# marcomistretta/incremental_multimodal_medical_learning_II

Hardware: AMD Instinct MI355X
Metric: contrastive train-step images/sec at global batch 1024; 1/2/4/8-GPU scaling (higher is better)
Workload: dtype bf16x3

## Files before the change

### incremental_multimodal_medical_learning_ii_amd/csrc/bert.hip

```cpp
#include "cxrk.h"
#include "cxrk_common.h"
#include "dropout.h"

using namespace cxrk;

namespace {

constexpr int LN_MAXV = 16;

template <bool EMBED>
__global__ __launch_bounds__(256) void ln_fwd_kernel(const float* __restrict__ x, const float* __restrict__ res,
                                                     const long* __restrict__ ids, const float* __restrict__ word,
                                                     const float* __restrict__ pos, const float* __restrict__ type,
                                                     const float* __restrict__ gamma, const float* __restrict__ beta,
                                                     float eps, long rows, int H, int L, float* __restrict__ y,
                                                     float* __restrict__ xhat, float* __restrict__ rstd_out) {
  const long row = (long)blockIdx.x * 4 + (threadIdx.x >> 6);
  if (row >= rows) return;
  const int lane = threadIdx.x & 63;
  float v[LN_MAXV];
  float s = 0.f;
  const float* xr = EMBED ? word + ids[row] * H : x + row * H;
  const float* rr = EMBED ? pos + (row % L) * H : (res ? res + row * H : nullptr);
#pragma unroll
// ... 317 lines not shown
    const int row = i / d4, c4 = i % d4;
    *reinterpret_cast<float4*>(Qs + row * ALD + c4 * 4) = *reinterpret_cast<const float4*>(base + (long)row * ld + c4 * 4);
    *reinterpret_cast<float4*>(Ks + row * ALD + c4 * 4) = *reinterpret_cast<const float4*>(base + (long)row * ld + nH * dH + c4 * 4);
    *reinterpret_cast<float4*>(Vs + row * ALD + c4 * 4) = *reinterpret_cast<const float4*>(base + (long)row * ld + 2 * nH * dH + c4 * 4);
  }
  __syncthreads();
  const int LP = L + 1;
  const int nb = (L + 1) / 2;
  for (int blk = threadIdx.x; blk < nb * nb; blk += 256) {
    const int i0 = 2 * (blk / nb), j0 = 2 * (blk % nb);
    const int i1 = min(i0 + 1, L - 1), j1 = min(j0 + 1, L - 1);
    float o[2][2];
    dot2x2(Qs, Ks, ALD, d4, i0, i1, j0, j1, o);
    const bool m0 = mask && mask[(long)b * L + j0] == 0, m1 = mask && mask[(long)b * L + j1] == 0;
    constexpr float MASKED = -3.4028234663852886e38f;
    Ps[i0 * LP + j0] = m0 ? MASKED : o[0][0] * scale;
    Ps[i0 * LP + j1] = m1 ? MASKED : o[0][1] * scale;
    Ps[i1 * LP + j0] = m0 ? MASKED : o[1][0] * scale;
    Ps[i1 * LP + j1] = m1 ? MASKED : o[1][1] * scale;
  }
  __syncthreads();
  {
    const int row = threadIdx.x >> 2, sub = threadIdx.x & 3;
    if (row < L) {
      float m = -INFINITY;
      for (int j = sub; j < L; j += 4) m = fmaxf(m, Ps[row * LP + j]);
      m = fmaxf(m, __shfl_xor(m, 1, 64)); m = fmaxf(m, __shfl_xor(m, 2, 64));
      float sum = 0.f;
      for (int j = sub; j < L; j += 4) { const float p = expf(Ps[row * LP + j] - m); Ps[row * LP + j] = p; sum += p; }
      sum += __shfl_xor(sum, 1, 64); sum += __shfl_xor(sum, 2, 64);
      const float inv = 1.0f / sum;
      for (int j = sub; j < L; j += 4) {
        const float p = Ps[row * LP + j] * inv;
        Ps[row * LP + j] = p;
        if (probs) probs[(((long)b * nH + hd) * L + row) * L + j] = p;
      }
    }
  }
  __syncthreads();
  if constexpr (DROP) {
    const int nj4 = (L + 3) / 4;
    for (int e = threadIdx.x; e < L * nj4; e += 256)
      drop_prob_row4(dk, Ps + (e / nj4) * LP, 0, e % nj4, L, (unsigned)(dk.row_offset + b), e / nj4, hd);
    __syncthreads();
  }
  const long obase = (long)b * L * (nH * dH) + hd * dH;
  float* out = ctx + obase;
  for (int blk = threadIdx.x; blk < nb * d4; blk += 256) {
    const int i0 = 2 * (blk / d4), dq = blk % d4;
    const int i1 = min(i0 + 1, L - 1);
    float4 a0 = make_float4(0.f, 0.f, 0.f, 0.f), a1 = a0;
    for (int j = 0; j < L; ++j) {
      const float4 v = *reinterpret_cast<const float4*>(Vs + j * ALD + dq * 4);
      fma4(a0, Ps[i0 * LP + j], v); fma4(a1, Ps[i1 * LP + j], v);
    }
    if (ctxp) {
      const float v0[4] = {a0.x, a0.y, a0.z, a0.w}, v1[4] = {a1.x, a1.y, a1.z, a1.w};
      planes_store4(ctxp, ctxplane, obase + (long)i0 * (nH * dH) + dq * 4, v0);
      if (i0 + 1 < L) planes_store4(ctxp, ctxplane, obase + (long)i1 * (nH * dH) + dq * 4, v1);
    } else {
      *reinterpret_cast<float4*>(out + (long)i0 * (nH * dH) + dq * 4) = a0;
      if (i0 + 1 < L) *reinterpret_cast<float4*>(out + (long)i1 * (nH * dH) + dq * 4) = a1;
    }
  }
}

template <bool DROP = false>
__global__ __launch_bounds__(256) void attn_bwd_kernel(const float* __restrict__ qkv, const float* __restrict__ probs,
                                                       const float* __restrict__ dctx, int L, int nH, int dH, float scale,
                                                       float* __restrict__ dqkv, unsigned short* __restrict__ dqkvp, long dqkvplane,
                                                       DropKey dk) {
  extern __shared__ __attribute__((aligned(16))) float smem[];
  const int ALD = dH + 4;
  float* Qs = smem; float* Ks = Qs + L * ALD; float* Vs = Ks + L * ALD; float* Os = Vs + L * ALD;
  float* Ps = Os + L * ALD; float* Ds = Ps + L * (L + 1);
  float* Pv = DROP ? Ds + L * (L + 1) : Ps;
  const int b = blockIdx.x / nH, hd = blockIdx.x % nH;
  const int ld = 3 * nH * dH;
  const int d4 = dH / 4;
  const float* base = qkv + (long)b * L * ld + hd * dH;
  const float* dob = dctx + (long)b * L * (nH * dH) + hd * dH;
  for (int i = threadIdx.x; i < L * d4; i += 256) {
    const int row = i / d4, c4 = i % d4;
    *reinterpret_cast<float4*>(Qs + row * ALD + c4 * 4) = *reinterpret_cast<const float4*>(base + (long)row * ld + c4 * 4);
    *reinterpret_cast<float4*>(Ks + row * ALD + c4 * 4) = *reinterpret_cast<const float4*>(base + (long)row * ld + nH * dH + c4 * 4);
    *reinterpret_cast<float4*>(Vs + row * ALD + c4 * 4) = *reinterpret_cast<const float4*>(base + (long)row * ld + 2 * nH * dH + c4 * 4);
    *reinterpret_cast<float4*>(Os + row * ALD + c4 * 4) = *reinterpret_cast<const float4*>(dob + (long)row * (nH * dH) + c4 * 4);
  }
  const int LP = L + 1;
  const float* pb = probs + ((long)b * nH + hd) * L * L;
  for (int e = threadIdx.x; e < L * L; e += 256) Ps[(e / L) * LP + (e % L)] = pb[e];
  __syncthreads();
  const int nb = (L + 1) / 2;
  for (int blk = threadIdx.x; blk < nb * nb; blk += 256) {
    const int i0 = 2 * (blk / nb), j0 = 2 * (blk % nb);
    const int i1 = min(i0 + 1, L - 1), j1 = min(j0 + 1, L - 1);
    float o[2][2];
    dot2x2(Os, Vs, ALD, d4, i0, i1, j0, j1, o);
    Ds[i0 * LP + j0] = o[0][0]; Ds[i0 * LP + j1] = o[0][1]; Ds[i1 * LP + j0] = o[1][0]; Ds[i1 * LP + j1] = o[1][1];
  }
  __syncthreads();
  if constexpr (DROP) {
    const int nj4 = (L + 3) / 4;
    for (int e = threadIdx.x; e < L * nj4; e += 256) {
      const int row = e / nj4, g = e % nj4;
      float f[4];
      drop_factors4(dk, (unsigned)g, (unsigned)(dk.row_offset + b), (unsigned)row | ((unsigned)hd << 16), f);
#pragma unroll
      for (int q = 0; q < 4; ++q) {
        const int j = 4 * g + q;
        if (j < L) { Ds[row * LP + j] *= f[q]; Pv[row * LP + j] = Ps[row * LP + j] * f[q]; }
      }
    }
    __syncthreads();
  }
  {
    const int row = threadIdx.x >> 2, sub = threadIdx.x & 3;
    if (row < L) {
      float t = 0.f;
      for (int j = sub; j < L; j += 4) t += Ds[row * LP + j] * Ps[row * LP + j];
      t += __shfl_xor(t, 1, 64); t += __shfl_xor(t, 2, 64);
      for (int j = sub; j < L; j += 4) Ds[row * LP + j] = Ps[row * LP + j] * (Ds[row * LP + j] - t) * scale;
    }
  }
  __syncthreads();
  const long qbase = (long)b * L * ld + hd * dH;
  float* dq = dqkv + qbase;
  auto put = [&](long off, const float4& v) {
    if (dqkvp) { const float t[4] = {v.x, v.y, v.z, v.w}; planes_store4(dqkvp, dqkvplane, qbase + off, t); }
    else *reinterpret_cast<float4*>(dq + off) = v;
  };
  for (int blk = threadIdx.x; blk < nb * d4; blk += 256) {
    const int i0 = 2 * (blk / d4), c = blk % d4;
    const int i1 = min(i0 + 1, L - 1);
    const float4 z = make_float4(0.f, 0.f, 0.f, 0.f);
    float4 q0 = z, q1 = z, k0 = z, k1 = z, v0 = z, v1 = z;
    for (int j = 0; j < L; ++j) {
      const float4 kj = *reinterpret_cast<const float4*>(Ks + j * ALD + c * 4);
      const float4 qj = *reinterpret_cast<const float4*>(Qs + j * ALD + c * 4);
      const float4 oj = *reinterpret_cast<const float4*>(Os + j * ALD + c * 4);
      fma4(q0, Ds[i0 * LP + j], kj); fma4(q1, Ds[i1 * LP + j], kj);
      fma4(k0, Ds[j * LP + i0], qj); fma4(k1, Ds[j * LP + i1], qj);
      fma4(v0, Pv[j * LP + i0], oj); fma4(v1, Pv[j * LP + i1], oj);
    }
    const long o0 = (long)i0 * ld + c * 4;
    put(o0, q0); put(o0 + nH * dH, k0); put(o0 + 2 * nH * dH, v0);
    if (i0 + 1 < L) {
      const long o1 = (long)i1 * ld + c * 4;
      put(o1, q1); put(o1 + nH * dH, k1); put(o1 + 2 * nH * dH, v1);
    }
  }
}

constexpr int ALONG = 512;
constexpr int TQ = 32, TK = 64;

__device__ __forceinline__ void load_rows(float* dst, const float* src, long ld, int r0, int nrows, int L, int d4, int ALD) {
  for (int i = threadIdx.x; i < nrows * d4; i += 256) {
    const int row = i / d4, c4 = i % d4;
    float4 v = make_float4(0.f, 0.f, 0.f, 0.f);
    if (r0 + row < L) v = *reinterpret_cast<const float4*>(src + (long)(r0 + row) * ld + c4 * 4);
    *reinterpret_cast<float4*>(dst + row * ALD + c4 * 4) = v;
  }
}
__device__ __forceinline__ void dot1x8(const float* X, const float* Y, int ALD, int d4n, int i, int jg, float (&o)[8]) {
#pragma unroll
  for (int c = 0; c < 8; ++c) o[c] = 0.f;
  const float4* x = reinterpret_cast<const float4*>(X + i * ALD);
  for (int d = 0; d < d4n; ++d) {
    const float4 a = x[d];
#pragma unroll
    for (int c = 0; c < 8; ++c) o[c] = dot4(a, reinterpret_cast<const float4*>(Y + (jg + 8 * c) * ALD)[d], o[c]);
  }
}

template <bool DROP = false>
__global__ __launch_bounds__(256) void attn_fwd_long_kernel(const float* __restrict__ qkv, const long* __restrict__ mask, int L, int nH,
                                                            int dH, float scale, float* __restrict__ ctx,
                                                            unsigned short* __restrict__ ctxp, long ctxplane, float* __restrict__ probs,
                                                            DropKey dk) {
  extern __shared__ __attribute__((aligned(16))) float smem[];
  const int ALD = dH + 4, d4 = dH / 4, LP = L + 1;
  float* Qs = smem; float* Ts = Qs + TQ * ALD; float* Ps = Ts + TK * ALD;
  const int nqt = (L + TQ - 1) / TQ;
  const int qt = blockIdx.x % nqt, bh = blockIdx.x / nqt;
  const int b = bh / nH, hd = bh % nH;
  const int ld = 3 * nH * dH;
  const float* base = qkv + (long)b * L * ld + hd * dH;
  const int q0 = qt * TQ;
  const int i = threadIdx.x >> 3, sub = threadIdx.x & 7;
  constexpr float MASKED = -3.4028234663852886e38f;
  load_rows(Qs, base, ld, q0, TQ, L, d4, ALD);
  for (int k0 = 0; k0 < L; k0 += TK) {
    __syncthreads();
    load_rows(Ts, base + nH * dH, ld, k0, TK, L, d4, ALD);
    __syncthreads();
    float o[8];
    dot1x8(Qs, Ts, ALD, d4, i, sub, o);
#pragma unroll
    for (int c = 0; c < 8; ++c) {
      const int j = k0 + sub + 8 * c;
      if (j < L) Ps[i * LP + j] = (mask && mask[(long)b * L + j] == 0) ? MASKED : o[c] * scale;
    }
  }
  __syncthreads();
  {
    float m = -INFINITY;
    for (int j = sub; j < L; j += 8) m = fmaxf(m, Ps[i * LP + j]);
    m = fmaxf(m, __shfl_xor(m, 1, 64)); m = fmaxf(m, __shfl_xor(m, 2, 64)); m = fmaxf(m, __shfl_xor(m, 4, 64));
    float sum = 0.f;
    for (int j = sub; j < L; j += 8) { const float pv = expf(Ps[i * LP + j] - m); Ps[i * LP + j] = pv; sum += pv; }
    sum += __shfl_xor(sum, 1, 64); sum += __shfl_xor(sum, 2, 64); sum += __shfl_xor(sum, 4, 64);
    const float inv = 1.0f / sum;
    for (int j = sub; j < L; j += 8) {
      const float pv = Ps[i * LP + j] * inv;
      Ps[i * LP + j] = pv;
      if (probs && q0 + i < L) probs[(((long)b * nH + hd) * L + q0 + i) * L + j] = pv;
    }
  }
  if constexpr (DROP) {
    __syncthreads();
    if (q0 + i < L)
      for (int g = sub; 4 * g < L; g += 8) drop_prob_row4(dk, Ps + i * LP, 0, g, L, (unsigned)(dk.row_offset + b), q0 + i, hd);
  }
  float4 acc[2] = {make_float4(0.f, 0.f, 0.f, 0.f), make_float4(0.f, 0.f, 0.f, 0.f)};
  for (int k0 = 0; k0 < L; k0 += TK) {
    __syncthreads();
    load_rows(Ts, base + 2 * nH * dH, ld, k0, TK, L, d4, ALD);
    __syncthreads();
    const int jn = min(TK, L - k0);
    for (int j = 0; j < jn; ++j) {
      const float pv = Ps[i * LP + k0 + j];
      if (sub < d4) fma4(acc[0], pv, *reinterpret_cast<const float4*>(Ts + j * ALD + sub * 4));
      if (sub + 8 < d4) fma4(acc[1], pv, *reinterpret_cast<const float4*>(Ts + j * ALD + (sub + 8) * 4));
    }
  }
  if (q0 + i < L) {
    const long obase = (long)b * L * (nH * dH) + hd * dH + (long)(q0 + i) * (nH * dH);
#pragma unroll
    for (int h = 0; h < 2; ++h) {
      const int dq = sub + 8 * h;
      if (dq >= d4) continue;
      if (ctxp) { const float v[4] = {acc[h].x, acc[h].y, acc[h].z, acc[h].w}; planes_store4(ctxp, ctxplane, obase + dq * 4, v); }
      else *reinterpret_cast<float4*>(ctx + obase + dq * 4) = acc[h];
    }
  }
}

__device__ __forceinline__ void drop_tile(const DropKey& dk, float* F, int q0, int k0, int L, unsigned n, int hd) {
  constexpr int G = TK / 4;
  for (int e = threadIdx.x; e < TQ * G; e += 256) {
    const int ii = e / G, g = e % G;
    float f[4] = {0.f, 0.f, 0.f, 0.f};
    if (q0 + ii < L) drop_factors4(dk, (unsigned)(k0 / 4 + g), n, (unsigned)(q0 + ii) | ((unsigned)hd << 16), f);
#pragma unroll
    for (int q = 0; q < 4; ++q) F[ii * (TK + 1) + 4 * g + q] = f[q];
  }
}

template <bool DROP = false>
__global__ __launch_bounds__(256) void attn_bwd_long_q_kernel(const float* __restrict__ qkv, const float* __restrict__ probs,
                                                              const float* __restrict__ dctx, int L, int nH, int dH, float scale,
                                                              float* __restrict__ dS, float* __restrict__ dqkv,
                                                              unsigned short* __restrict__ dqkvp, long dqkvplane, DropKey dk) {
  extern __shared__ __attribute__((aligned(16))) float smem[];
  const int ALD = dH + 4, d4 = dH / 4, DP = TK + 1;
  float* Os = smem; float* Ks = Os + TQ * ALD; float* Vs = Ks + TK * ALD; float* Ds = Vs + TK * ALD;
  const int nqt = (L + TQ - 1) / TQ;
  const int qt = blockIdx.x % nqt, bh = blockIdx.x / nqt;
  const int b = bh / nH, hd = bh % nH;
  const int ld = 3 * nH * dH;
  const float* base = qkv + (long)b * L * ld + hd * dH;
  const float* dob = dctx + (long)b * L * (nH * dH) + hd * dH;
  const float* pb = probs + ((long)b * nH + hd) * L * L;
  float* dsb = dS + ((long)b * nH + hd) * L * L;
  const int q0 = qt * TQ;
  const int i = threadIdx.x >> 3, sub = threadIdx.x & 7;
  const bool rowok = q0 + i < L;
  load_rows(Os, dob, nH * dH, q0, TQ, L, d4, ALD);
  float t = 0.f;
  for (int k0 = 0; k0 < L; k0 += TK) {
    __syncthreads();
    load_rows(Vs, base + 2 * nH * dH, ld, k0, TK, L, d4, ALD);
    if constexpr (DROP) drop_tile(dk, Ds, q0, k0, L, (unsigned)(dk.row_offset + b), hd);
    __syncthreads();
    float o[8];
    dot1x8(Os, Vs, ALD, d4, i, sub, o);
#pragma unroll
    for (int c = 0; c < 8; ++c) {
      const int j = k0 + sub + 8 * c;
      if constexpr (DROP) o[c] *= Ds[i * DP + sub + 8 * c];
      if (rowok && j < L) t = fmaf(pb[(long)(q0 + i) * L + j], o[c], t);
    }
  }
  t += __shfl_xor(t, 1, 64); t += __shfl_xor(t, 2, 64); t += __shfl_xor(t, 4, 64);
  float4 acc[2] = {make_float4(0.f, 0.f, 0.f, 0.f), make_float4(0.f, 0.f, 0.f, 0.f)};
  for (int k0 = 0; k0 < L; k0 += TK) {
    __syncthreads();
    load_rows(Ks, base + nH * dH, ld, k0, TK, L, d4, ALD);
    load_rows(Vs, base + 2 * nH * dH, ld, k0, TK, L, d4, ALD);
    if constexpr (DROP) drop_tile(dk, Ds, q0, k0, L, (unsigned)(dk.row_offset + b), hd);
    __syncthreads();
    float o[8];
    dot1x8(Os, Vs, ALD, d4, i, sub, o);
#pragma unroll
    for (int c = 0; c < 8; ++c) {
// ... 87 lines not shown
        planes_store4(dqkvp, dqkvplane, koff + nH * dH + dq * 4, a);
        planes_store4(dqkvp, dqkvplane, koff + 2 * nH * dH + dq * 4, c);
      } else {
        *reinterpret_cast<float4*>(dqkv + koff + nH * dH + dq * 4) = dk[h];
        *reinterpret_cast<float4*>(dqkv + koff + 2 * nH * dH + dq * 4) = dv[h];
      }
    }
  }
}

__global__ void planes_add_rows_kernel(const unsigned short* __restrict__ src, long plane, long rows, int cols, float* __restrict__ dst,
                                       long ld) {
  const int c8n = cols / 8;
  for (long i = (long)blockIdx.x * blockDim.x + threadIdx.x; i < rows * c8n; i += (long)gridDim.x * blockDim.x) {
    const long r = i / c8n; const int c = (int)(i - r * c8n) * 8;
    float v[8]; planes_load8(src, plane, r * cols + c, v);
    float* d = dst + r * ld + c;
    float4 a = *reinterpret_cast<float4*>(d), b = *reinterpret_cast<float4*>(d + 4);
    a.x += v[0]; a.y += v[1]; a.z += v[2]; a.w += v[3]; b.x += v[4]; b.y += v[5]; b.z += v[6]; b.w += v[7];
    *reinterpret_cast<float4*>(d) = a; *reinterpret_cast<float4*>(d + 4) = b;
  }
}

__global__ void gelu_bwd_kernel(const float* __restrict__ dy, const float* __restrict__ pre, long n, float* __restrict__ dx) {
  const long i = (long)blockIdx.x * blockDim.x + threadIdx.x;
  if (i < n) dx[i] = dy[i] * gelu_erf_grad(pre[i]);
}

}

extern "C" int cxrk_planes_add_rows(const void* src, long plane, long rows, int cols, float* dst, long ld, hipStream_t stream) {
  CXRK_CHECK_ARG(src && dst && rows > 0 && cols > 0 && (cols % 8) == 0 && (plane % 8) == 0 && (ld % 4) == 0 && aligned16(src) && aligned16(dst));
  long nb = (rows * (cols / 8) + 255) / 256; if (nb > 2048) nb = 2048;
  hipLaunchKernelGGL(planes_add_rows_kernel, dim3((unsigned)nb), dim3(256), 0, stream, static_cast<const unsigned short*>(src), plane, rows,
                     cols, dst, ld);
  CXRK_LAUNCH_CHECK();
  return CXRK_OK;
}

extern "C" int cxrk_gelu_bwd(const float* dy, const float* pre, long n, float* dx, hipStream_t stream) {
  CXRK_CHECK_ARG(dy && pre && dx && n > 0);
  hipLaunchKernelGGL(gelu_bwd_kernel, dim3((unsigned)((n + 255) / 256)), dim3(256), 0, stream, dy, pre, n, dx);
  CXRK_LAUNCH_CHECK();
  return CXRK_OK;
}

static bool ln_vec8_ok(int H, const void* a, const void* b, const void* c, const void* d, const void* e, const void* f) {
  return (H % 8) == 0 && aligned16(a) && aligned16(b) && aligned16(c) && aligned16(d) && aligned16(e) && aligned16(f);
}


template <bool EMBED, bool DROP>
static int launch_ln_fwd(const float* x, const float* res, const long* ids, const float* word, const float* pos, const float* type,
                         const float* gamma, const float* beta, float eps, long rows, int H, int L, void* y, long yplane, float* xhat,
                         float* rstd, bool v8, const LnFwdDrop& dr, hipStream_t stream) {
  const dim3 grid((unsigned)((rows + 3) / 4));
  if (v8 || DROP)
    hipLaunchKernelGGL((ln_fwd_vec8_kernel<EMBED, DROP>), grid, dim3(256), 0, stream, x, res, ids, word, pos, type, gamma, beta, eps, rows, H,
                       L, yplane ? nullptr : static_cast<float*>(y), yplane ? static_cast<unsigned short*>(y) : nullptr, yplane, xhat, rstd,
                       dr);
  else
    hipLaunchKernelGGL((ln_fwd_kernel<EMBED>), grid, dim3(256), 0, stream, x, res, ids, word, pos, type, gamma, beta, eps, rows, H, L,
                       static_cast<float*>(y), xhat, rstd);
  CXRK_LAUNCH_CHECK();
  return CXRK_OK;
}

extern "C" int cxrk_embed_ln_fwd(const long* ids, const float* word, const float* pos, const float* type,
                                 const float* gamma, const float* beta, float eps, long T, int L, int H, void* y, long yplane,
                                 float* xhat, float* rstd, hipStream_t stream) {
  CXRK_CHECK_ARG(ids && word && pos && type && gamma && beta && y && T > 0 && L > 0 && H > 0 && H <= 64 * LN_MAXV && yplane >= 0);
  const bool v8 = ln_vec8_ok(H, word, pos, type, gamma, beta, y) && aligned16(xhat) && (yplane % 8) == 0;
  if (yplane > 0 && !v8) return CXRK_ERR_ARG;
  return launch_ln_fwd<true, false>(nullptr, nullptr, ids, word, pos, type, gamma, beta, eps, T, H, L, y, yplane, xhat, rstd, v8,
                                    LnFwdDrop{}, stream);
}

extern "C" int cxrk_residual_ln_fwd(const float* x, const float* res, const float* gamma, const float* beta, float eps,
                                    long rows, int H, void* y, long yplane, float* xhat, float* rstd, hipStream_t stream) {
  CXRK_CHECK_ARG(x && gamma && beta && y && rows > 0 && H > 0 && H <= 64 * LN_MAXV && yplane >= 0);
  const bool v8 = ln_vec8_ok(H, x, res, gamma, beta, y, xhat) && (yplane % 8) == 0;
  if (yplane > 0 && !v8) return CXRK_ERR_ARG;
  return launch_ln_fwd<false, false>(x, res, nullptr, nullptr, nullptr, nullptr, gamma, beta, eps, rows, H, 1, y, yplane, xhat, rstd, v8,
                                     LnFwdDrop{}, stream);
}

static int ln_bwd_blocks(long rows) {
  long nb = (rows + 15) / 16;
  if (nb > 1024) nb = 1024;
  if (nb < 1) nb = 1;
  return (int)nb;
}
extern "C" size_t cxrk_residual_ln_bwd_ws_bytes(long rows, int H) { return (size_t)ln_bwd_blocks(rows) * 3 * H * sizeof(float); }

static bool ln_bwd_vec_ok(int H, const float* dy, const float* xhat, const float* gamma, const void* dxv, const float* dx_add, long dxplane) {
  return (H % 4 == 0) && aligned16(dy) && aligned16(xhat) && aligned16(gamma) && aligned16(dxv) && (!dx_add || aligned16(dx_add)) &&
         (dxplane % 4) == 0;
}

template <int DM>
static int launch_ln_bwd(const float* dy, const float* xhat, const float* rstd, const float* gamma, long rows, int H, const float* dx_add,
                         void* dxv, long dxplane, float* dgamma, float* dbeta, int accumulate, float* dxsum, int dxsum_accumulate, float* ws,
                         bool vec, const LnBwdDrop& dr, hipStream_t stream) {
  float* dx = dxplane ? nullptr : static_cast<float*>(dxv);
  unsigned short* dxp = dxplane ? static_cast<unsigned short*>(dxv) : nullptr;
  int nb = ln_bwd_blocks(rows);
  const int np = dxsum ? 3 : 2;
  const int rows_per = (int)((rows + nb - 1) / nb);
  nb = (int)((rows + rows_per - 1) / rows_per);
  if (vec || DM != LNB_PLAIN)
    hipLaunchKernelGGL(ln_bwd_vec_kernel<DM>, dim3(nb), dim3(256), 0, stream, dy, xhat, rstd, gamma, rows, H, rows_per, dx, dxp, dxplane, dx_add,
                       ws, np, dr);
  else
    hipLaunchKernelGGL(ln_bwd_kernel, dim3(nb), dim3(256), 0, stream, dy, xhat, rstd, gamma, rows, H, rows_per, dx, dx_add, ws);
  CXRK_LAUNCH_CHECK();
  hipLaunchKernelGGL(ln_bwd_final_kernel, dim3(ceil_div(H, 64), np), dim3(1024), 0, stream, ws, nb, np, H, dgamma, dbeta, accumulate, dxsum,
                     dxsum_accumulate);
  CXRK_LAUNCH_CHECK();
  return CXRK_OK;
}

extern "C" int cxrk_residual_ln_bwd(const float* dy, const float* xhat, const float* rstd, const float* gamma, long rows,
                                    int H, const float* dx_add, void* dxv, long dxplane, float* dgamma, float* dbeta, int accumulate,
                                    float* dxsum, int dxsum_accumulate, float* ws, size_t ws_bytes, hipStream_t stream) {
  CXRK_CHECK_ARG(dy && xhat && rstd && gamma && dxv && dgamma && dbeta && rows > 0 && H > 0 && H <= 64 * LN_MAXV && dxplane >= 0);
  CXRK_CHECK_WS(ws, ws_bytes, cxrk_residual_ln_bwd_ws_bytes(rows, H));
  const bool vec = ln_bwd_vec_ok(H, dy, xhat, gamma, dxv, dx_add, dxplane);
  if ((dxplane || dxsum) && !vec) return CXRK_ERR_ARG;
  return launch_ln_bwd<LNB_PLAIN>(dy, xhat, rstd, gamma, rows, H, dx_add, dxv, dxplane, dgamma, dbeta, accumulate, dxsum, dxsum_accumulate, ws,
                                  vec, LnBwdDrop{}, stream);
}

template <bool DROP>
static int launch_attn_fwd(const float* qkv, const long* mask, int B, int L, int nH, int dH, void* ctxv, long ctxplane, float* probs,
                           const DropKey& dk, hipStream_t stream) {
  float* ctx = ctxplane ? nullptr : static_cast<float*>(ctxv);
  unsigned short* ctxp = ctxplane ? static_cast<unsigned short*>(ctxv) : nullptr;
  if (dH > AD || dH < 4 || (dH % 4) != 0 || L > ALONG || L < 1) return CXRK_ERR_UNSUPPORTED;
  const int ALD = dH + 4;
  const float scale = 1.0f / sqrtf((float)dH);
  if (L > AL) {
    const size_t shl = (size_t)((TQ + TK) * ALD + TQ * (L + 1)) * sizeof(float);
    static bool attr_long = false;
    if (!attr_long) {
      (void)hipFuncSetAttribute(reinterpret_cast<const void*>(attn_fwd_long_kernel<DROP>), hipFuncAttributeMaxDynamicSharedMemorySize,
                                (int)(((TQ + TK) * (AD + 4) + TQ * (ALONG + 1)) * sizeof(float)));
      attr_long = true;
    }
    hipLaunchKernelGGL(attn_fwd_long_kernel<DROP>, dim3((unsigned)(B * nH * ceil_div(L, TQ))), dim3(256), shl, stream, qkv, mask, L, nH, dH,
                       scale, ctx, ctxp, ctxplane, probs, dk);
    CXRK_LAUNCH_CHECK();
    return CXRK_OK;
  }
  const size_t sh = (size_t)(3 * L * ALD + L * (L + 1)) * sizeof(float);
  static bool attr_set = false;
  if (!attr_set) {
    (void)hipFuncSetAttribute(reinterpret_cast<const void*>(attn_fwd_kernel<DROP>), hipFuncAttributeMaxDynamicSharedMemorySize,
                              (int)((3 * AL * (AD + 4) + AL * (AL + 1)) * sizeof(float)));
    attr_set = true;
  }
  hipLaunchKernelGGL(attn_fwd_kernel<DROP>, dim3((unsigned)(B * nH)), dim3(256), sh, stream, qkv, mask, L, nH, dH, scale, ctx, ctxp, ctxplane,
                     probs, dk);
  CXRK_LAUNCH_CHECK();
  return CXRK_OK;
}

extern "C" int cxrk_attn_fwd(const float* qkv, const long* mask, int B, int L, int nH, int dH, void* ctxv, long ctxplane, float* probs,
                             hipStream_t stream) {
  CXRK_CHECK_ARG(qkv && ctxv && B > 0 && nH > 0 && aligned16(qkv) && aligned16(ctxv) && ctxplane >= 0 && (ctxplane % 4) == 0);
  return launch_attn_fwd<false>(qkv, mask, B, L, nH, dH, ctxv, ctxplane, probs, DropKey{}, stream);
}

extern "C" size_t cxrk_attn_bwd_ws_bytes(int B, int L, int nH, int dH) {
  (void)dH;
  return L > AL ? (size_t)B * nH * L * L * sizeof(float) : 0;
}

template <bool DROP>
static int launch_attn_bwd(const float* qkv, const float* probs, const float* dctx, int B, int L, int nH, int dH, void* dqkvv, long dqkvplane,
                           float* ws, size_t ws_bytes, const DropKey& dk, hipStream_t stream) {
  float* dqkv = dqkvplane ? nullptr : static_cast<float*>(dqkvv);
  unsigned short* dqkvp = dqkvplane ? static_cast<unsigned short*>(dqkvv) : nullptr;
  if (dH > AD || dH < 4 || (dH % 4) != 0 || L > ALONG || L < 1) return CXRK_ERR_UNSUPPORTED;
  const int ALD = dH + 4;
  const float scale = 1.0f / sqrtf((float)dH);
  if (L > AL) {
    CXRK_CHECK_WS(ws, ws_bytes, cxrk_attn_bwd_ws_bytes(B, L, nH, dH));
    const size_t shq = (size_t)((TQ + 2 * TK) * ALD + TQ * (TK + 1)) * sizeof(float);
    const size_t shk = (size_t)(2 * TQ * ALD + 2 * TQ * (TK + 1)) * sizeof(float);
    hipLaunchKernelGGL(attn_bwd_long_q_kernel<DROP>, dim3((unsigned)(B * nH * ceil_div(L, TQ))), dim3(256), shq, stream, qkv, probs, dctx, L,
                       nH, dH, scale, ws, dqkv, dqkvp, dqkvplane, dk);
    CXRK_LAUNCH_CHECK();
    hipLaunchKernelGGL(attn_bwd_long_kv_kernel<DROP>, dim3((unsigned)(B * nH * ceil_div(L, TK))), dim3(256), shk, stream, qkv, probs, ws, dctx,
                       L, nH, dH, dqkv, dqkvp, dqkvplane, dk);
    CXRK_LAUNCH_CHECK();
    return CXRK_OK;
  }
  constexpr int NP = DROP ? 3 : 2;
  const size_t sh = (size_t)(4 * L * ALD + NP * L * (L + 1)) * sizeof(float);
  static bool attr_set = false;
  if (!attr_set) {
    (void)hipFuncSetAttribute(reinterpret_cast<const void*>(attn_bwd_kernel<DROP>), hipFuncAttributeMaxDynamicSharedMemorySize,
                              (int)((4 * AL * (AD + 4) + NP * AL * (AL + 1)) * sizeof(float)));
    attr_set = true;
  }
  hipLaunchKernelGGL(attn_bwd_kernel<DROP>, dim3((unsigned)(B * nH)), dim3(256), sh, stream, qkv, probs, dctx, L, nH, dH, scale, dqkv, dqkvp,
                     dqkvplane, dk);
  CXRK_LAUNCH_CHECK();
  return CXRK_OK;
}

extern "C" int cxrk_attn_bwd(const float* qkv, const float* probs, const float* dctx, int B, int L, int nH, int dH,
                             void* dqkvv, long dqkvplane, float* ws, size_t ws_bytes, hipStream_t stream) {
  CXRK_CHECK_ARG(qkv && probs && dctx && dqkvv && B > 0 && nH > 0 && aligned16(qkv) && aligned16(dctx) && aligned16(dqkvv) && dqkvplane >= 0 &&
                 (dqkvplane % 4) == 0);
  return launch_attn_bwd<false>(qkv, probs, dctx, B, L, nH, dH, dqkvv, dqkvplane, ws, ws_bytes, DropKey{}, stream);
}

namespace {

__global__ __launch_bounds__(256) void dropout_mask_kernel(DropKey dk, int N, int L, int nH, int C, unsigned char* __restrict__ keep) {
  const int C4 = (C + 3) / 4;
  const long total = (long)N * nH * L * C4;
  for (long e = (long)blockIdx.x * blockDim.x + threadIdx.x; e < total; e += (long)gridDim.x * blockDim.x) {
    const int g = (int)(e % C4);
    const long r = e / C4;
    const int t = (int)(r % L), h = (int)((r / L) % nH), n = (int)(r / ((long)L * nH));
    float f[4];
    drop_factors4(dk, (unsigned)g, (unsigned)(dk.row_offset + n), (unsigned)t | ((unsigned)h << 16), f);
#pragma unroll
    for (int q = 0; q < 4; ++q)
      if (4 * g + q < C) keep[r * C + 4 * g + q] = f[q] != 0.f;
  }
}

}

static int make_drop(unsigned long long seed, unsigned counter, int layer, int site, long row_offset, float p, int rows_per_seq,
                     DropKey& d) {
  if (!(p >= 0.f && p < 1.f) || layer < 0 || layer > 63 || site < 0 || site > 3 || row_offset < 0 || rows_per_seq < 1) return CXRK_ERR_ARG;
  d.k0 = (unsigned)(seed & 0xffffffffull);
  d.k1 = (unsigned)(seed >> 32);
  d.c3 = ((counter & 0xffffffu) << 8) | ((unsigned)layer << 2) | (unsigned)site;
  d.thresh = (unsigned)floor((double)p * 4294967296.0 + 0.5);
  d.scale = 1.0f / (1.0f - p);
  d.row_offset = row_offset;
  d.rows_per_seq = rows_per_seq;
  return CXRK_OK;
}
#define CXRK_MAKE_DROP(rps, d)                                                              \
  DropKey d;                                                                                \
  if (make_drop(seed, counter, layer, site, row_offset, p, (rps), d) != CXRK_OK) return CXRK_ERR_ARG

extern "C" int cxrk_dropout_mask(unsigned long long seed, unsigned counter, int layer, int site, long row_offset, float p, int N, int L,
                                 int nH, int C, unsigned char* keep, hipStream_t stream) {
  CXRK_CHECK_ARG(keep && N > 0 && L > 0 && nH > 0 && nH < 65536 && L < 65536 && C > 0);
  CXRK_MAKE_DROP(1, dk);
  long nb = ((long)N * nH * L * ((C + 3) / 4) + 255) / 256;
  if (nb > 4096) nb = 4096;
  hipLaunchKernelGGL(dropout_mask_kernel, dim3((unsigned)nb), dim3(256), 0, stream, dk, N, L, nH, C, keep);
  CXRK_LAUNCH_CHECK();
  return CXRK_OK;
}

extern "C" int cxrk_embed_ln_fwd_drop(const long* ids, const float* word, const float* pos, const float* type, const float* gamma,
                                      const float* beta, float eps, long T, int L, int H, void* y, long yplane, float* xhat, float* rstd,
                                      unsigned long long seed, unsigned counter, int layer, int site, long row_offset, float p,
                                      hipStream_t stream) {
  CXRK_CHECK_ARG(ids && word && pos && type && gamma && beta && y && T > 0 && L > 0 && H > 0 && H <= 64 * LN_MAXV && yplane >= 0);
  if (!(ln_vec8_ok(H, word, pos, type, gamma, beta, y) && aligned16(xhat) && (yplane % 8) == 0)) return CXRK_ERR_UNSUPPORTED;
  LnFwdDrop dr{};
  if (make_drop(seed, counter, layer, site, row_offset, p, L, dr.dk) != CXRK_OK) return CXRK_ERR_ARG;
  return launch_ln_fwd<true, true>(nullptr, nullptr, ids, word, pos, type, gamma, beta, eps, T, H, L, y, yplane, xhat, rstd, true, dr, stream);
}

extern "C" int cxrk_residual_ln_fwd_drop(const float* x, const void* res, long resplane, long res_ld, const float* gamma, const float* beta,
                                         float eps, long rows, int H, int rows_per_seq, void* y, long yplane, float* xhat, float* rstd,
                                         unsigned long long seed, unsigned counter, int layer, int site, long row_offset, float p,
                                         hipStream_t stream) {
  CXRK_CHECK_ARG(x && gamma && beta && y && rows > 0 && H > 0 && H <= 64 * LN_MAXV && yplane >= 0 && resplane >= 0 && res_ld >= 0);
  if (!(ln_vec8_ok(H, x, res, gamma, beta, y, xhat) && (yplane % 8) == 0 && (resplane % 8) == 0 && (res_ld % 8) == 0))
    return CXRK_ERR_UNSUPPORTED;
  LnFwdDrop dr{};
  if (make_drop(seed, counter, layer, site, row_offset, p, rows_per_seq, dr.dk) != CXRK_OK) return CXRK_ERR_ARG;
  dr.resp = resplane ? static_cast<const unsigned short*>(res) : nullptr;
  dr.resplane = resplane;
  dr.res_ld = res_ld ? res_ld : H;
  return launch_ln_fwd<false, true>(x, resplane ? nullptr : static_cast<const float*>(res), nullptr, nullptr, nullptr, nullptr, gamma, beta,
                                    eps, rows, H, 1, y, yplane, xhat, rstd, true, dr, stream);
}

extern "C" int cxrk_residual_ln_bwd_drop(const float* dy, const float* xhat, const float* rstd, const float* gamma, long rows, int H,
                                         int rows_per_seq, int mode, const float* dx_add, void* dxv, void* dxmv, long dxplane, float* dgamma,
                                         float* dbeta, int accumulate, float* dxsum, int dxsum_accumulate, float* ws, size_t ws_bytes,
                                         unsigned long long seed, unsigned counter, int layer, int site, long row_offset, float p,
                                         hipStream_t stream) {
  CXRK_CHECK_ARG(dy && xhat && rstd && gamma && dxv && dgamma && dbeta && rows > 0 && H > 0 && H <= 64 * LN_MAXV && dxplane >= 0 &&
                 (mode == LNB_DROP_RES || mode == LNB_DROP_DY) && ((mode == LNB_DROP_RES) == (dxmv != nullptr)));
  CXRK_CHECK_WS(ws, ws_bytes, cxrk_residual_ln_bwd_ws_bytes(rows, H));
  if (!(ln_bwd_vec_ok(H, dy, xhat, gamma, dxv, dx_add, dxplane) && (!dxmv || aligned16(dxmv)))) return CXRK_ERR_UNSUPPORTED;
  LnBwdDrop dr{};
  if (make_drop(seed, counter, layer, site, row_offset, p, rows_per_seq, dr.dk) != CXRK_OK) return CXRK_ERR_ARG;
  dr.dxm = dxplane ? nullptr : static_cast<float*>(dxmv);
  dr.dxmp = dxplane ? static_cast<unsigned short*>(dxmv) : nullptr;
  return mode == LNB_DROP_RES
             ? launch_ln_bwd<LNB_DROP_RES>(dy, xhat, rstd, gamma, rows, H, dx_add, dxv, dxplane, dgamma, dbeta, accumulate, dxsum,
                                           dxsum_accumulate, ws, true, dr, stream)
             : launch_ln_bwd<LNB_DROP_DY>(dy, xhat, rstd, gamma, rows, H, dx_add, dxv, dxplane, dgamma, dbeta, accumulate, dxsum,
                                          dxsum_accumulate, ws, true, dr, stream);
}

extern "C" int cxrk_attn_fwd_drop(const float* qkv, const long* mask, int B, int L, int nH, int dH, void* ctxv, long ctxplane, float* probs,
                                  unsigned long long seed, unsigned counter, int layer, int site, long row_offset, float p,
                                  hipStream_t stream) {
  CXRK_CHECK_ARG(qkv && ctxv && B > 0 && nH > 0 && nH < 65536 && aligned16(qkv) && aligned16(ctxv) && ctxplane >= 0 && (ctxplane % 4) == 0);
  CXRK_MAKE_DROP(1, dk);
  return launch_attn_fwd<true>(qkv, mask, B, L, nH, dH, ctxv, ctxplane, probs, dk, stream);
}

extern "C" int cxrk_attn_bwd_drop(const float* qkv, const float* probs, const float* dctx, int B, int L, int nH, int dH, void* dqkvv,
                                  long dqkvplane, float* ws, size_t ws_bytes, unsigned long long seed, unsigned counter, int layer, int site,
                                  long row_offset, float p, hipStream_t stream) {
  CXRK_CHECK_ARG(qkv && probs && dctx && dqkvv && B > 0 && nH > 0 && nH < 65536 && aligned16(qkv) && aligned16(dctx) && aligned16(dqkvv) &&
                 dqkvplane >= 0 && (dqkvplane % 4) == 0);
  CXRK_MAKE_DROP(1, dk);
  return launch_attn_bwd<true>(qkv, probs, dctx, B, L, nH, dH, dqkvv, dqkvplane, ws, ws_bytes, dk, stream);
}
```

Measured before the change: 6879.

## Add MFMA-based attention forward/backward kernels for short sequences with dH=64

Adds single-wavefront attention kernels that use fp32 32x32x2 MFMA instructions for QK^T, PV and the backward gradient products when L<=32 and head dim is 64. The kernels run as a persistent grid sized from the CU count, and each block prefetches the next head's Q/K/V (and dO/P) into registers while computing the current one. The aim is to replace the scalar-FMA shared-memory attention for the short text sequences. The new path is on by default and can be turned off with an environment variable. It adds register pressure and duplicates the softmax and dropout logic.

```diff
diff --git a/incremental_multimodal_medical_learning_ii_amd/csrc/attn_mfma.h b/incremental_multimodal_medical_learning_ii_amd/csrc/attn_mfma.h
--- /dev/null
+++ b/incremental_multimodal_medical_learning_ii_amd/csrc/attn_mfma.h
@@ -0,0 +1,310 @@
+constexpr int MALD = 68;
+constexpr int MLP = 36;
+constexpr int ML = 32;
+
+static inline bool attn_mfma_enabled() { const char* e = getenv("CXRK_ATTN_MFMA"); return e ? atoi(e) != 0 : true; }
+static inline bool attn_mfma_shape(int L, int dH) { return dH == 64 && L >= 1 && L <= ML; }
+
+constexpr int MFMA_FWD_RESIDENT = 6, MFMA_BWD_RESIDENT = 4;
+static inline int attn_mfma_cus() {
+  static const int n = [] { int dev = 0, v = 0; if (hipGetDevice(&dev) != hipSuccess || hipDeviceGetAttribute(&v, hipDeviceAttributeMultiprocessorCount, dev) != hipSuccess || v <= 0) v = 256; return v; }();
+  return n;
+}
+static inline unsigned attn_mfma_grid(long nheads, int resident) { const long cap = (long)attn_mfma_cus() * resident; return (unsigned)(nheads < cap ? nheads : cap); }
+
+__device__ __forceinline__ int cd_row(int g, int h) { return (g & 3) + 8 * (g >> 2) + 4 * h; }
+
+struct MfmaRows { float4 v[ML * 16 / 64]; };
+__device__ __forceinline__ void mfma_fetch(MfmaRows& t, const float* src, long ld, int L, int lane) {
+#pragma unroll
+  for (int it = 0; it < ML * 16 / 64; ++it) {
+    const int row = min(it * 4 + (lane >> 4), L - 1), c4 = lane & 15;
+    t.v[it] = *reinterpret_cast<const float4*>(src + (long)row * ld + c4 * 4);
+  }
+}
+__device__ __forceinline__ void mfma_stage(float* dst, const MfmaRows& t, int L, int lane) {
+#pragma unroll
+  for (int it = 0; it < ML * 16 / 64; ++it) {
+    const int row = it * 4 + (lane >> 4), c4 = lane & 15;
+    *reinterpret_cast<float4*>(dst + row * MALD + c4 * 4) = row < L ? t.v[it] : make_float4(0.f, 0.f, 0.f, 0.f);
+  }
+}
+
+__device__ __forceinline__ f32x16 mfma_xyT(const float* X, const float* Y, int r, int h) {
+  f32x16 acc = {0.f, 0.f, 0.f, 0.f, 0.f, 0.f, 0.f, 0.f, 0.f, 0.f, 0.f, 0.f, 0.f, 0.f, 0.f, 0.f};
+  const float4* x = reinterpret_cast<const float4*>(X + r * MALD);
+  const float4* y = reinterpret_cast<const float4*>(Y + r * MALD);
+#pragma unroll
+  for (int q = 0; q < 16; ++q) {
+    const float4 a = x[q], b = y[q];
+    acc = __builtin_amdgcn_mfma_f32_32x32x2f32(h ? a.z : a.w, h ? b.z : b.w, acc, 0, 0, 0);
+    acc = __builtin_amdgcn_mfma_f32_32x32x2f32(h ? a.x : a.y, h ? b.x : b.y, acc, 0, 0, 0);
+  }
+  return acc;
+}
+
+__device__ __forceinline__ void mfma_row_a(const float* A, const float* Y, int L, int r, int h, f32x16& acc0, f32x16& acc1) {
+  const float4* a4 = reinterpret_cast<const float4*>(A + r * MLP);
+  const int nq = (L + 3) >> 2;
+  for (int q = 0; q < nq; ++q) {
+    const float4 p = a4[q];
+    const float* y0 = Y + (4 * q + h) * MALD + r;
+    const float* y1 = y0 + 2 * MALD;
+    acc0 = __builtin_amdgcn_mfma_f32_32x32x2f32(h ? p.y : p.x, y0[0], acc0, 0, 0, 0);
+    acc1 = __builtin_amdgcn_mfma_f32_32x32x2f32(h ? p.y : p.x, y0[32], acc1, 0, 0, 0);
+    acc0 = __builtin_amdgcn_mfma_f32_32x32x2f32(h ? p.w : p.z, y1[0], acc0, 0, 0, 0);
+    acc1 = __builtin_amdgcn_mfma_f32_32x32x2f32(h ? p.w : p.z, y1[32], acc1, 0, 0, 0);
+  }
+}
+
+template <int LDA>
+__device__ __forceinline__ void mfma_col_a(const float* A, const float* Y, int L, int r, int h, f32x16& acc0, f32x16& acc1) {
+  const int ns = (L + 1) >> 1;
+  for (int s = 0; s < ns; ++s) {
+    const float a = A[(2 * s + h) * LDA + r];
+    const float* y = Y + (2 * s + h) * MALD + r;
+    acc0 = __builtin_amdgcn_mfma_f32_32x32x2f32(a, y[0], acc0, 0, 0, 0);
+    acc1 = __builtin_amdgcn_mfma_f32_32x32x2f32(a, y[32], acc1, 0, 0, 0);
+  }
+}
+
+__device__ __forceinline__ void mfma_unload(float* St, const f32x16& acc0, const f32x16& acc1, int r, int h) {
+#pragma unroll
+  for (int g = 0; g < 16; ++g) {
+    St[cd_row(g, h) * MALD + r] = acc0[g];
+    St[cd_row(g, h) * MALD + 32 + r] = acc1[g];
+  }
+}
+
+template <bool DROP>
+__global__ __launch_bounds__(64) void attn_fwd_mfma_kernel(const float* __restrict__ qkv, const long* __restrict__ mask, int nheads, int Larg,
+                                                           int nH, float scale, float* __restrict__ ctx, unsigned short* __restrict__ ctxp,
+                                                           long ctxplane, float* __restrict__ probs, DropKey dk) {
+  constexpr int dH = 64;
+  __shared__ __attribute__((aligned(16))) float smem[3 * ML * MALD];
+  float* Qs = smem; float* Ks = Qs + ML * MALD; float* Vs = Ks + ML * MALD;
+  float* Ps = Qs;
+  float* Cs = Ks;
+  const int lane = threadIdx.x, r = lane & 31, h = lane >> 5;
+  const int ld = 3 * nH * dH;
+  MfmaRows q, k, v;
+  bool mnext = false;
+  auto fetch = [&](int head) {
+    const int b = head / nH, hd = head % nH;
+    const float* base = qkv + (long)b * Larg * ld + hd * dH;
+    mnext = mask && mask[(long)b * Larg + min(r, Larg - 1)] == 0;
+    mfma_fetch(q, base, ld, Larg, lane);
+    mfma_fetch(k, base + nH * dH, ld, Larg, lane);
+    mfma_fetch(v, base + 2 * nH * dH, ld, Larg, lane);
+  };
+  fetch(blockIdx.x);
+  for (int head = blockIdx.x; head < nheads; head += gridDim.x) {
+  int L = Larg;
+  asm volatile("" : "+s"(L));
+  const int b = head / nH, hd = head % nH;
+  const bool mj = mnext && r < L;
+  mfma_stage(Qs, q, L, lane); mfma_stage(Ks, k, L, lane); mfma_stage(Vs, v, L, lane);
+  if (head + (int)gridDim.x < nheads) fetch(head + gridDim.x);
+  __syncthreads();
+  const f32x16 s = mfma_xyT(Qs, Ks, r, h);
+  __syncthreads();
+  constexpr int LP = MLP;
+  {
+    constexpr float MASKED = -3.4028234663852886e38f;
+#pragma unroll
+    for (int g = 0; g < 16; ++g) {
+      const int i = cd_row(g, h);
+      Ps[i * LP + r] = (i < L && r < L) ? (mj ? MASKED : s[g] * scale) : -0.f;
+    }
+  }
+  __syncthreads();
+  {
+    const int sub = lane & 3;
+#pragma unroll
+    for (int rr = 0; rr < ML / 16; ++rr) {
+      const int row = 16 * rr + (lane >> 2);
+      if (row < L) {
+        float v[ML / 4];
+#pragma unroll
+        for (int c = 0; c < ML / 4; ++c) v[c] = sub + 4 * c < L ? Ps[row * LP + sub + 4 * c] : -INFINITY;
+        float m = -INFINITY;
+#pragma unroll
+        for (int c = 0; c < ML / 4; ++c) m = fmaxf(m, v[c]);
+        m = fmaxf(m, __shfl_xor(m, 1, 64)); m = fmaxf(m, __shfl_xor(m, 2, 64));
+        float sum = 0.f;
+#pragma unroll
+        for (int c = 0; c < ML / 4; ++c)
+          if (sub + 4 * c < L) { const float p = expf(v[c] - m); v[c] = p; sum += p; }
+        sum += __shfl_xor(sum, 1, 64); sum += __shfl_xor(sum, 2, 64);
+        const float inv = 1.0f / sum;
+#pragma unroll
+        for (int c = 0; c < ML / 4; ++c)
+          if (sub + 4 * c < L) Ps[row * LP + sub + 4 * c] = v[c] * inv;
+      }
+    }
+  }
+  __syncthreads();
+  if (probs) {
+    float* pb = probs + ((long)b * nH + hd) * L * L;
+#pragma unroll 4
+    for (int it = 0; it < ML * ML / 64; ++it) {
+      const int i = 2 * it + h;
+      if (i < L && r < L) pb[i * L + r] = Ps[i * LP + r];
+    }
+  }
+  if constexpr (DROP) {
+    __syncthreads();
+    DropKey dkh = dk;
+    asm volatile("" : "+s"(dkh.k0), "+s"(dkh.k1));
+    const int nj4 = (L + 3) / 4;
+    for (int e = lane; e < L * nj4; e += 64)
+      drop_prob_row4(dkh, Ps + (e / nj4) * LP, 0, e % nj4, L, (unsigned)(dkh.row_offset + b), e / nj4, hd);
+    __syncthreads();
+  }
+  f32x16 c0 = {0.f, 0.f, 0.f, 0.f, 0.f, 0.f, 0.f, 0.f, 0.f, 0.f, 0.f, 0.f, 0.f, 0.f, 0.f, 0.f}, c1 = c0;
+  mfma_row_a(Ps, Vs, L, r, h, c0, c1);
+  mfma_unload(Cs, c0, c1, r, h);
+  __syncthreads();
+  const long obase = (long)b * L * (nH * dH) + hd * dH;
+#pragma unroll 2
+  for (int it = 0; it < ML * 16 / 64; ++it) {
+    const int row = it * 4 + (lane >> 4), c4 = lane & 15;
+    if (row < L) {
+      const float4 v = *reinterpret_cast<const float4*>(Cs + row * MALD + c4 * 4);
+      const long off = obase + (long)row * (nH * dH) + c4 * 4;
+      if (ctxp) { const float t[4] = {v.x, v.y, v.z, v.w}; planes_store4(ctxp, ctxplane, off, t); }
+      else *reinterpret_cast<float4*>(ctx + off) = v;
+    }
+  }
+  __syncthreads();
+  }
+}
+
+template <bool DROP>
+__global__ __launch_bounds__(64) void attn_bwd_mfma_kernel(const float* __restrict__ qkv, const float* __restrict__ probs,
+                                                           const float* __restrict__ dctx, int nheads, int Larg, int nH, float scale,
+                                                           float* __restrict__ dqkv, unsigned short* __restrict__ dqkvp, long dqkvplane,
+                                                           DropKey dk) {
+  constexpr int dH = 64;
+  constexpr int PVLD = DROP ? ML : MLP;
+  static_assert(ML * MLP + ML * ML <= ML * MALD, "dS and the dropped P replace V");
+  __shared__ __attribute__((aligned(16))) float smem[4 * ML * MALD + ML * MLP];
+  float* Qs = smem; float* Ks = Qs + ML * MALD; float* Vs = Ks + ML * MALD; float* Os = Vs + ML * MALD;
+  float* Ps = Os + ML * MALD;
+  float* Ds = Vs;
+  float* Pv = DROP ? Ds + ML * MLP : Ps;
+  const int lane = threadIdx.x, r = lane & 31, h = lane >> 5;
+  const int ld = 3 * nH * dH;
+  MfmaRows o, v, q, k;
+  float p[ML * ML / 64];
+  auto fetch = [&](int head) {
+    const int b = head / nH, hd = head % nH;
+    const float* base = qkv + (long)b * Larg * ld + hd * dH;
+    mfma_fetch(o, dctx + (long)b * Larg * (nH * dH) + hd * dH, nH * dH, Larg, lane);
+    mfma_fetch(v, base + 2 * nH * dH, ld, Larg, lane);
+    const float* pb = probs + ((long)b * nH + hd) * Larg * Larg;
+#pragma unroll
+    for (int it = 0; it < ML * ML / 64; ++it) p[it] = pb[min(2 * it + h, Larg - 1) * Larg + min(r, Larg - 1)];
+    mfma_fetch(q, base, ld, Larg, lane);
+    mfma_fetch(k, base + nH * dH, ld, Larg, lane);
+  };
+  fetch(blockIdx.x);
+  for (int head = blockIdx.x; head < nheads; head += gridDim.x) {
+  int L = Larg;
+  asm volatile("" : "+s"(L));
+  const int b = head / nH, hd = head % nH;
+  mfma_stage(Os, o, L, lane); mfma_stage(Vs, v, L, lane);
+#pragma unroll
+  for (int it = 0; it < ML * ML / 64; ++it) Ps[(2 * it + h) * MLP + r] = (2 * it + h < L && r < L) ? p[it] : -0.f;
+  mfma_stage(Qs, q, L, lane); mfma_stage(Ks, k, L, lane);
+  if (head + (int)gridDim.x < nheads) fetch(head + gridDim.x);
+  __syncthreads();
+  constexpr int LP = MLP;
+  {
+    const f32x16 dp = mfma_xyT(Os, Vs, r, h);
+    __syncthreads();
+#pragma unroll
+    for (int g = 0; g < 16; ++g) {
+      const int i = cd_row(g, h);
+      Ds[i * LP + r] = (i < L && r < L) ? dp[g] : -0.f;
+    }
+    if constexpr (DROP) {
+#pragma unroll 4
+      for (int it = 0; it < ML * ML / 64; ++it) Pv[(2 * it + h) * PVLD + r] = -0.f;
+    }
+  }
+  __syncthreads();
+  if constexpr (DROP) {
+    const int nj4 = (L + 3) / 4;
+    for (int e = lane; e < L * nj4; e += 64) {
+      const int row = e / nj4, g = e % nj4;
+      float f[4];
+      drop_factors4(dk, (unsigned)g, (unsigned)(dk.row_offset + b), (unsigned)row | ((unsigned)hd << 16), f);
+#pragma unroll
+      for (int q = 0; q < 4; ++q) {
+        const int j = 4 * g + q;
+        if (j < L) { Ds[row * LP + j] *= f[q]; Pv[row * PVLD + j] = Ps[row * LP + j] * f[q]; }
+      }
+    }
+    __syncthreads();
+  }
+  {
+    const int sub = lane & 3;
+#pragma unroll
+    for (int rr = 0; rr < ML / 16; ++rr) {
+      const int row = 16 * rr + (lane >> 2);
+      if (row < L) {
+        float d[ML / 4], pr[ML / 4];
+#pragma unroll
+        for (int c = 0; c < ML / 4; ++c) {
+          const bool in = sub + 4 * c < L;
+          d[c] = in ? Ds[row * LP + sub + 4 * c] : 0.f;
+          pr[c] = in ? Ps[row * LP + sub + 4 * c] : 0.f;
+        }
+        float t = 0.f;
+#pragma unroll
+        for (int c = 0; c < ML / 4; ++c)
+          if (sub + 4 * c < L) t += d[c] * pr[c];
+        t += __shfl_xor(t, 1, 64); t += __shfl_xor(t, 2, 64);
+#pragma unroll
+        for (int c = 0; c < ML / 4; ++c)
+          if (sub + 4 * c < L) Ds[row * LP + sub + 4 * c] = pr[c] * (d[c] - t) * scale;
+      }
+    }
+  }
+  __syncthreads();
+  const long qbase = (long)b * L * ld + hd * dH;
+  auto emit = [&](float* St, const f32x16& a0, const f32x16& a1, int col) {
+    __syncthreads();
+    mfma_unload(St, a0, a1, r, h);
+    __syncthreads();
+#pragma unroll 2
+    for (int it = 0; it < ML * 16 / 64; ++it) {
+      const int row = it * 4 + (lane >> 4), c4 = lane & 15;
+      if (row < L) {
+        const float4 v = *reinterpret_cast<const float4*>(St + row * MALD + c4 * 4);
+        const long off = qbase + (long)row * ld + col + c4 * 4;
+        if (dqkvp) { const float t[4] = {v.x, v.y, v.z, v.w}; planes_store4(dqkvp, dqkvplane, off, t); }
+        else *reinterpret_cast<float4*>(dqkv + off) = v;
+      }
+    }
+  };
+  const f32x16 z = {0.f, 0.f, 0.f, 0.f, 0.f, 0.f, 0.f, 0.f, 0.f, 0.f, 0.f, 0.f, 0.f, 0.f, 0.f, 0.f};
+  {
+    f32x16 a0 = z, a1 = z;
+    mfma_col_a<PVLD>(Pv, Os, L, r, h, a0, a1);
+    emit(Os, a0, a1, 2 * nH * dH);
+  }
+  {
+    f32x16 a0 = z, a1 = z;
+    mfma_col_a<MLP>(Ds, Qs, L, r, h, a0, a1);
+    emit(Qs, a0, a1, nH * dH);
+  }
+  {
+    f32x16 a0 = z, a1 = z;
+    mfma_row_a(Ds, Ks, L, r, h, a0, a1);
+    emit(Ks, a0, a1, 0);
+  }
+  __syncthreads();
+  }
+}
diff --git a/incremental_multimodal_medical_learning_ii_amd/csrc/bert.hip b/incremental_multimodal_medical_learning_ii_amd/csrc/bert.hip
--- a/incremental_multimodal_medical_learning_ii_amd/csrc/bert.hip
+++ b/incremental_multimodal_medical_learning_ii_amd/csrc/bert.hip
@@ -493,6 +493,8 @@
   }
 }
 
+#include "attn_mfma.h"
+
 constexpr int ALONG = 512;
 constexpr int TQ = 32, TK = 64;
 
@@ -886,6 +888,12 @@
     CXRK_LAUNCH_CHECK();
     return CXRK_OK;
   }
+  if (attn_mfma_shape(L, dH) && attn_mfma_enabled()) {
+    hipLaunchKernelGGL(attn_fwd_mfma_kernel<DROP>, dim3(attn_mfma_grid((long)B * nH, MFMA_FWD_RESIDENT)), dim3(64), 0, stream, qkv, mask, B * nH, L, nH, scale, ctx, ctxp, ctxplane,
+                       probs, dk);
+    CXRK_LAUNCH_CHECK();
+    return CXRK_OK;
+  }
   const size_t sh = (size_t)(3 * L * ALD + L * (L + 1)) * sizeof(float);
   static bool attr_set = false;
   if (!attr_set) {
@@ -930,6 +938,12 @@
     CXRK_LAUNCH_CHECK();
     return CXRK_OK;
   }
+  if (attn_mfma_shape(L, dH) && attn_mfma_enabled()) {
+    hipLaunchKernelGGL(attn_bwd_mfma_kernel<DROP>, dim3(attn_mfma_grid((long)B * nH, MFMA_BWD_RESIDENT)), dim3(64), 0, stream, qkv, probs, dctx, B * nH, L, nH, scale, dqkv, dqkvp,
+                       dqkvplane, dk);
+    CXRK_LAUNCH_CHECK();
+    return CXRK_OK;
+  }
   constexpr int NP = DROP ? 3 : 2;
   const size_t sh = (size_t)(4 * L * ALD + NP * L * (L + 1)) * sizeof(float);
   static bool attr_set = false;
```

After: 6904, median of 6. Within noise of the previous version (+0.4%).
